# UCSB-NLP-Chang/Diffusion-SpaceTime-Attn

Measured on AMD Instinct MI355X. Metric: images/sec at 512x512, 50 PLMS steps, 2 objects, higher is better.
Workload: dtype fp16; 1 GPU; SD-v1-4 UNet+VAE (synthetic weights), 512x512, 50 PLMS steps (51 CFG UNet calls), 2 objects, fixed blend weights (BASELINE configs[1]); global_batch=64, parallelism=prompt-parallel dp1, hipgraph=True, linear_weights=fp16, trunk_layout=NHWC, weight_broadcast_bytes=0

## Files before the change

### diffusion-spacetime-attn_amd/csrc/sta_gemm.hip

```cpp

#include <hip/hip_runtime.h>
#include <stdint.h>
#include <type_traits>
#include "sta_xattn.h"
#include "sta_unet.h"
#include "sta_internal.h"
#include "sta_xattn_dev.h"

namespace {

constexpr int GM_NW = 8;
constexpr int GM_ROWS = 256;
constexpr int gm_part(int ntw) { return 32 * ntw; }
constexpr int gm_nt(int ntw) { return 2 * ntw; }
constexpr int gm_wfr(int ntw) { return 2 * gm_nt(ntw); }
constexpr int gm_wper(int ntw) { return (gm_wfr(ntw) + GM_NW - 1) / GM_NW; }
constexpr int gm_wslot(int ntw) { return gm_wper(ntw) * GM_NW * FRAG; }
constexpr int GM_XPER = 2 * (GM_ROWS / 16) / GM_NW;
constexpr int GM_XBUF = 2 * GM_ROWS * 64;
constexpr int gm_lds(int ntw) { return 2 * gm_wslot(ntw) + 2 * GM_XBUF; }

template <typename T>
__global__ __launch_bounds__(64) void pack_gemm_w_kernel(const T* __restrict__ w, long sn, long sk, T* __restrict__ packed, int nsteps, int nt) {
  const int fr = blockIdx.x;
  const int t = fr % nt, kci = (fr / nt) & 1, step = (fr / (2 * nt)) % nsteps, part = fr / (2 * nt * nsteps);
  const int lane = threadIdx.x, g = lane >> 4, c = lane & 15;
  const T* src = w + (size_t)(16 * nt * part + 16 * t + c) * sn + (size_t)(64 * step + 32 * kci + 8 * g) * sk;
  typename Tr<T>::V8 x;
#pragma unroll
  for (int j = 0; j < 8; ++j) x[j] = src[j * sk];
  *(typename Tr<T>::V8*)(packed + (size_t)fr * (FRAG / 2) + lane * 8) = x;
}

__device__ __forceinline__ float gm_row16_sum(float x) {
  x += __builtin_bit_cast(float, __builtin_amdgcn_update_dpp(0, __builtin_bit_cast(int, x), 0xB1, 0xf, 0xf, true));
  x += __builtin_bit_cast(float, __builtin_amdgcn_update_dpp(0, __builtin_bit_cast(int, x), 0x4E, 0xf, 0xf, true));
  x += __builtin_bit_cast(float, __builtin_amdgcn_update_dpp(0, __builtin_bit_cast(int, x), 0x141, 0xf, 0xf, true));
  x += __builtin_bit_cast(float, __builtin_amdgcn_update_dpp(0, __builtin_bit_cast(int, x), 0x140, 0xf, 0xf, true));
  return x;
}

struct GM {
  const char* x;
  const char* xb;
  int Ka;
  const char* w;
  const char* zeros;
  void* out;
  const void* bias;
  const void* res;
  float* stats;
  long rows_img;
  long R;
  int K, N, parts, items, xcd_map;
  long tiles;
};

template <typename T, int NTW>
__global__ __launch_bounds__(64 * GM_NW, 1) void gemm_rows_kernel(const GM p) {
  using V8 = typename Tr<T>::V8;
  using V4 = typename Tr<T>::V4;
  constexpr int PART = gm_part(NTW), NT = gm_nt(NTW), WFR = gm_wfr(NTW), WPER = gm_wper(NTW), WSLOT = gm_wslot(NTW);
  const int lane = threadIdx.x & 63;
  const int wv = __builtin_amdgcn_readfirstlane(threadIdx.x >> 6);
  const int g = lane >> 4, c16 = lane & 15;
  const int pq = wv & 3, ch = wv >> 2;
  char* xring = smem;
  char* wring = smem + 2 * GM_XBUF;
  const int nsteps = p.K >> 6;
  const __amdgpu_buffer_rsrc_t w_srd = make_srd(p.w, (unsigned)((size_t)p.parts * nsteps * WFR * FRAG));
  const unsigned lane16 = (unsigned)lane * 16u;

  auto item_tile = [&](int it, long& tile, int& part) {
    if (p.xcd_map) {
      const int j = it >> 3;
      tile = (long)(j / p.parts) * 8 + (it & 7);
      part = j % p.parts;
    } else {
      tile = it / p.parts;
      part = it - (int)tile * p.parts;
    }
  };
  const int nsteps_a = p.xb ? p.Ka >> 6 : nsteps;
  auto in_ptr = [&](long tile, int pc, bool second) -> const char* {
    const int rl = 16 * (pc & 15) + (lane >> 2);
    const long row = tile * GM_ROWS + rl;
    const int chunk = (lane & 3) ^ (((rl >> 2) & 1) << 1);
    const char* base = second ? p.xb + (size_t)row * (p.K - p.Ka) * sizeof(T) : p.x + (size_t)row * (p.xb ? p.Ka : p.K) * sizeof(T);
    return row < p.R ? base + (pc >> 4) * 64 + chunk * 16 : p.zeros + (pc >> 4) * 64 + chunk * 16;
  };
  auto stage_w = [&](int part, int step, int slot) __attribute__((always_inline)) {
    const unsigned base = (unsigned)((part * nsteps + step) * WFR) * (unsigned)FRAG;
#pragma unroll
    for (int i = 0; i < WPER; ++i) {
      const int f = wv + GM_NW * i;
      const int fs = f < WFR ? f : 0;
      __builtin_amdgcn_raw_ptr_buffer_load_lds(w_srd, (__attribute__((address_space(3))) void*)(wring + slot * WSLOT + f * FRAG), 16, lane16,
                                               base + (unsigned)fs * (unsigned)FRAG, 0, 0);
    }
  };
  auto stage_x = [&](const char* src, int pc, int buf) __attribute__((always_inline)) {
    __builtin_amdgcn_global_load_lds((const __attribute__((address_space(1))) void*)src,
                                     (__attribute__((address_space(3))) void*)(xring + buf * GM_XBUF + pc * FRAG), 16, 0, 0);
  };
  unsigned seg_e[4];
#pragma unroll
  for (int q = 0; q < 4; ++q) {
    const int rl = 64 * pq + 16 * q + c16;
    seg_e[q] = (unsigned)(rl * 64 + ((g ^ (((rl >> 2) & 1) << 1)) << 4));
  }

// ... 39 lines not shown
      auto stage_next = [&]() __attribute__((always_inline)) {
        if (!last) stage_w(part, st + 1, SL ^ 1);
        else if (more) stage_w(npart, 0, SL ^ 1);
        if (!last || more) {
#pragma unroll
          for (int i = 0; i < GM_XPER; ++i) {
            if (last) xp[i] = in_ptr(ntile, wv + GM_NW * i, false);
            else if (st + 1 == nsteps_a) xp[i] = in_ptr(tile, wv + GM_NW * i, true);
            stage_x(xp[i], wv + GM_NW * i, SL ^ 1);
            xp[i] += 128;
          }
        }
      };
      const char* xb = xring + SL * GM_XBUF;
      const V8* wf = (const V8*)(wring + SL * WSLOT + lane * 16) + (NTW * ch) * 64;
      V8 a[NTW], b[4];
      auto load_kc = [&](int kci, V8 (&aa)[NTW], V8 (&bb)[4]) __attribute__((always_inline)) {
#pragma unroll
        for (int q = 0; q < 4; ++q) bb[q] = *(const V8*)(xb + kci * (GM_ROWS * 64) + seg_e[q]);
#pragma unroll
        for (int t = 0; t < NTW; ++t) aa[t] = wf[(kci * NT + t) * 64];
      };
      load_kc(0, a, b);
#pragma unroll
      for (int kci = 0; kci < 2; ++kci) {
        V8 an[NTW], bn[4];
        if (kci < 1) load_kc(kci + 1, an, bn);
        __builtin_amdgcn_sched_barrier(0);
#pragma unroll
        for (int t = 0; t < NTW; ++t)
#pragma unroll
          for (int q = 0; q < 4; ++q) acc[q][t] = Tr<T>::mfma(a[t], b[q], acc[q][t]);
        __builtin_amdgcn_sched_barrier(0);
        if (kci == 0) {
          stage_next();
          __builtin_amdgcn_sched_barrier(0);
#pragma unroll
          for (int t = 0; t < NTW; ++t) a[t] = an[t];
#pragma unroll
          for (int q = 0; q < 4; ++q) b[q] = bn[q];
        }
      }
    };
    auto run_tile = [&](auto p0_tag) __attribute__((always_inline)) {
      constexpr int P0 = decltype(p0_tag)::value;
      for (int st = 0; st < nsteps; st += 2) {
        step(std::integral_constant<int, P0>{}, st);
        if (st + 1 < nsteps) step(std::integral_constant<int, P0 ^ 1>{}, st + 1);
      }
    };
    if (par == 0) run_tile(std::integral_constant<int, 0>{});
    else run_tile(std::integral_constant<int, 1>{});
    par ^= nsteps & 1;
    {
      typedef __attribute__((ext_vector_type(2))) unsigned u32x2;
      float bs[NTW][4];
#pragma unroll
      for (int t = 0; t < NTW; ++t) {
        V4 bv = {};
        if (p.bias) bv = *(const V4*)((const T*)p.bias + part * PART + ch * (16 * NTW) + 16 * t + 4 * g);
#pragma unroll
        for (int r = 0; r < 4; ++r) bs[t][r] = (float)bv[r];
      }
      float ssum[NTW][4], ssq[NTW][4];
#pragma unroll
      for (int t = 0; t < NTW; ++t)
#pragma unroll
        for (int r = 0; r < 4; ++r) { ssum[t][r] = 0.f; ssq[t][r] = 0.f; }
#pragma unroll
      for (int q = 0; q < 4; ++q) {
        const long row = tile * GM_ROWS + 64 * pq + 16 * q + c16;
        const bool ok = row < p.R;
        const unsigned base = (unsigned)(((size_t)row * p.N + part * PART + ch * (16 * NTW) + 4 * g) * sizeof(T));
        V4 rv[NTW];
        if (p.res) {
#pragma unroll
          for (int t = 0; t < NTW; ++t)
            rv[t] = __builtin_bit_cast(V4, __builtin_amdgcn_raw_buffer_load_b64(r_srd, ok ? base + (unsigned)(16 * t * sizeof(T)) : 0xfffffff0u, 0, 0));
        }
#pragma unroll
        for (int t = 0; t < NTW; ++t) {
          V4 o;
#pragma unroll
          for (int r = 0; r < 4; ++r) o[r] = (T)(acc[q][t][r] + bs[t][r] + (p.res ? (float)rv[t][r] : 0.f));
          __builtin_amdgcn_raw_buffer_store_b64(__builtin_bit_cast(u32x2, o), o_srd, ok ? base + (unsigned)(16 * t * sizeof(T)) : 0xfffffff0u, 0, 0);
          if (p.stats) {
#pragma unroll
            for (int r = 0; r < 4; ++r) {
              const float v = ok ? (float)o[r] : 0.f;
              ssum[t][r] += v;
              ssq[t][r] += v * v;
            }
          }
        }
      }
      if (p.stats) {
        const long row0 = tile * GM_ROWS;
        const bool live = row0 < p.R;
        const long img = live ? row0 / p.rows_img : p.R / p.rows_img;
        const int slot = live ? (int)((row0 - img * p.rows_img) / GM_ROWS) * 4 + pq : pq;
        const int slots = (int)(p.rows_img / GM_ROWS) * 4;
        float* dst = p.stats + (((size_t)img * slots + slot) * p.N + part * PART + ch * (16 * NTW) + 4 * g) * 2;
#pragma unroll
        for (int t = 0; t < NTW; ++t) {
          f32x4 lo, hi;
          lo[0] = gm_row16_sum(ssum[t][0]); lo[1] = gm_row16_sum(ssq[t][0]); lo[2] = gm_row16_sum(ssum[t][1]); lo[3] = gm_row16_sum(ssq[t][1]);
          hi[0] = gm_row16_sum(ssum[t][2]); hi[1] = gm_row16_sum(ssq[t][2]); hi[2] = gm_row16_sum(ssum[t][3]); hi[3] = gm_row16_sum(ssq[t][3]);
          if (c16 == 0) {
            *(f32x4*)(dst + 32 * t) = lo;
            *(f32x4*)(dst + 32 * t + 4) = hi;
          }
        }
      }
    }
    if (!more) break;
    it = nit; tile = ntile; part = npart;
    first_of_tile = true;
  }
  asm volatile("s_waitcnt vmcnt(0)" ::: "memory");
}

}

extern "C" {

static int gemm_ntw(int N) { return N > 0 && N % 160 == 0 ? 5 : (N > 0 && N % 128 == 0 ? 4 : 0); }

int sta_linear_rows_supported(long R, int K, int N) {
  if (R <= 0 || K <= 0 || K % 64 || gemm_ntw(N) == 0) return 0;
  if ((size_t)R * N * 2 >= 0xfffffff0ull) return 0;
  return 1;
}

size_t sta_linear_rows_packed_w_bytes(int K, int N) { return (K > 0 && K % 64 == 0 && gemm_ntw(N)) ? (size_t)N * K * 2 : 0; }

int sta_linear_rows_pack_w(const void* w, long sn, long sk, void* packed, int K, int N, int dtype, void* stream) {
  g_sta_err[0] = 0;
  if (!w || !packed) return sta_fail(STA_E_ARG, "null pointer");
  if (sta_linear_rows_packed_w_bytes(K, N) == 0) return sta_fail(STA_E_UNSUP, "linear_rows: K %% 64 == 0 and N %% 160 == 0 or N %% 128 == 0 (K=%d N=%d)", K, N);
  hipStream_t st = (hipStream_t)stream;
  const int nsteps = K / 64, nt = gm_nt(gemm_ntw(N));
  const unsigned nfr = (unsigned)(N / (16 * nt)) * nsteps * 2 * nt;
  return sta_by_dtype(dtype, [&](auto tag) {
    using T = decltype(tag);
    return sta_launch<pack_gemm_w_kernel<T>>("pack_gemm_w launch", dim3(nfr), dim3(64), 0, st, (const T*)w, sn, sk, (T*)packed, nsteps, nt);
  });
}

static int linear_rows_impl(const void* x, const void* xb, int Ka, const void* packed_w, const void* zeros, const void* bias, const void* res,
                            void* out, long R, int K, int N, int dtype, void* stream, float* stats = nullptr, long rows_img = 0) {
  g_sta_err[0] = 0;
  if (!x || !packed_w || !zeros || !out) return sta_fail(STA_E_ARG, "null pointer");
  if (xb && (Ka <= 0 || Ka >= K || Ka % 64)) return sta_fail(STA_E_ARG, "linear_rows_cat: Ka=%d of K=%d (need 0 < Ka < K, Ka %% 64 == 0)", Ka, K);
  if (!sta_linear_rows_supported(R, K, N)) return sta_fail(STA_E_UNSUP, "linear_rows: unsupported shape R=%ld K=%d N=%d", R, K, N);
  if (dtype != STA_BF16 && dtype != STA_F16) return sta_fail(STA_E_UNSUP, "dtype %d", dtype);
  const int ntw = gemm_ntw(N);
  if (stats && (rows_img <= 0 || rows_img % GM_ROWS || R % rows_img)) return sta_fail(STA_E_ARG, "linear_rows_stats: rows_per_image=%ld (need a multiple of 256 dividing R=%ld)", rows_img, R);
  GM p{(const char*)x, (const char*)xb, Ka, (const char*)packed_w, (const char*)zeros, out, bias, res, stats, rows_img, R, K, N, N / gm_part(ntw), 0, 0, (R + GM_ROWS - 1) / GM_ROWS};
  const long items = p.tiles * p.parts;
  if (items >= (1l << 30)) return sta_fail(STA_E_UNSUP, "linear_rows: too many tiles");
  p.items = (int)items;
  p.xcd_map = p.tiles % 8 == 0;
  const unsigned grid = (unsigned)(p.items < 256 ? p.items : 256);
  hipStream_t st = (hipStream_t)stream;
  return sta_by_dtype(dtype, [&](auto tag) {
    using T = decltype(tag);
    const char* const what = "linear_rows launch";
    if (ntw == 5) return sta_launch_lds<gemm_rows_kernel<T, 5>>(what, gm_lds(5), dim3(grid), dim3(64 * GM_NW), gm_lds(5), st, p);
    return sta_launch_lds<gemm_rows_kernel<T, 4>>(what, gm_lds(4), dim3(grid), dim3(64 * GM_NW), gm_lds(4), st, p);
  });
}

int sta_linear_rows(const void* x, const void* packed_w, const void* zeros, const void* bias, const void* res, void* out, long R, int K, int N,
                    int dtype, void* stream) {
  return linear_rows_impl(x, nullptr, 0, packed_w, zeros, bias, res, out, R, K, N, dtype, stream);
}

int sta_linear_rows_stats(const void* x, const void* packed_w, const void* zeros, const void* bias, const void* res, void* out, float* stats,
                          long rows_per_image, long R, int K, int N, int dtype, void* stream) {
  if (!stats) { g_sta_err[0] = 0; return sta_fail(STA_E_ARG, "null pointer"); }
  return linear_rows_impl(x, nullptr, 0, packed_w, zeros, bias, res, out, R, K, N, dtype, stream, stats, rows_per_image);
}

int sta_linear_rows_cat(const void* xa, const void* xb, int Ka, const void* packed_w, const void* zeros, const void* bias, const void* res,
                        void* out, long R, int K, int N, int dtype, void* stream) {
  if (!xb) { g_sta_err[0] = 0; return sta_fail(STA_E_ARG, "null pointer"); }
  return linear_rows_impl(xa, xb, Ka, packed_w, zeros, bias, res, out, R, K, N, dtype, stream);
}

}
```

### diffusion-spacetime-attn_amd/sta/fused.py

```python

import torch

from . import lib

_DT = {torch.bfloat16: lib.STA_BF16, torch.float16: lib.STA_F16}
ENABLED = True
_hold = 0
TRACKED = False


class held:

    def __enter__(self):
        global _hold
        _hold += 1

    def __exit__(self, *exc):
        global _hold
        _hold -= 1


class tracked:

    def __init__(self, on=True):
# ... 365 lines not shown
    if n_post.shape != (B, 4, Hh, Ww) or n_enc.shape != (B, 4, Hh, Ww):
        raise ValueError("vae_encode_step: noises must be [B, 4, h, w] = %s" % ((B, 4, Hh, Ww),))
    x = torch.empty((B, 4, Hh, Ww), dtype=torch.float32, device=h.device)
    z0 = torch.empty_like(x) if want_z0 else None
    xin = torch.empty((2 * B, 4, Hh, Ww), dtype=h.dtype, device=h.device) if want_xin else None
    lib.check(lib.load().sta_vae_encode_step(h.data_ptr(), qw.data_ptr(), qb.data_ptr(), n_post.data_ptr(), n_enc.data_ptr(), x.data_ptr(),
                                             _ptr(z0), _ptr(xin), B, Hh * Ww, float(scale_factor), float(sqrt_a), float(sqrt_1ma), _DT[h.dtype],
                                             _stream()), "sta_vae_encode_step")
    return x, z0, xin


CAT_IN_PLACE = True


def groupnorm_silu_cat(xa, xb, weight, bias, groups, eps, silu=True):
    B, Ca = xa.shape[0], xa.shape[1]
    C = Ca + xb.shape[1]
    HW = xa.numel() // (B * Ca)
    L = lib.load()
    y = torch.empty((B, C) + tuple(xa.shape[2:]), dtype=xa.dtype, device=xa.device, memory_format=torch.channels_last)
    sa, sb = (_producer_stats(xa), _producer_stats(xb)) if GN_STATS_FROM_PRODUCER else (None, None)
    if sa is not None and sb is not None:
        lib.check(L.sta_groupnorm_silu_nhwc_cstats(xa.data_ptr(), xb.data_ptr(), Ca, sa.data_ptr(), sb.data_ptr(), None, weight.data_ptr(),
                                                   bias.data_ptr(), y.data_ptr(), B, C, HW, groups, float(eps), int(bool(silu)), _DT[xa.dtype],
                                                   _stream()), "sta_groupnorm_silu_nhwc_cstats")
        return y
    ws = torch.empty(L.sta_groupnorm_nhwc_workspace_bytes(B, HW, groups) // 4, dtype=torch.float32, device=xa.device)
    lib.check(L.sta_groupnorm_silu_nhwc_cat(xa.data_ptr(), xb.data_ptr(), Ca, None, weight.data_ptr(), bias.data_ptr(), y.data_ptr(),
                                            ws.data_ptr(), B, C, HW, groups, float(eps), int(bool(silu)), _DT[xa.dtype], _stream()),
              "sta_groupnorm_silu_nhwc_cat")
    return y


def cat_supported(xa, xb, groups, skip_weight):
    if not (CAT_IN_PLACE and usable(xa) and is_nhwc(xa) and is_nhwc(xb) and xa.dtype == xb.dtype and xa.shape[0] == xb.shape[0]
            and xa.shape[2:] == xb.shape[2:]):
        return False
    Ca, C = xa.shape[1], xa.shape[1] + xb.shape[1]
    if Ca % 64 or C % 8 or C % groups or (C // groups < 8 and C // groups != 4) or C > 4096 or groups > 64:
        return False
    rows = xa.numel() // Ca
    return (LINEAR_ROWS and rows >= LINEAR_MIN_ROWS and skip_weight.dtype == xa.dtype
            and bool(lib.load().sta_linear_rows_supported(rows, C, skip_weight.shape[0])))


def linear_rows_cat(xa, xb, w_packed, N, bias=None, res=None):
    Ka, Kb = xa.shape[-1], xb.shape[-1]
    R = xa.numel() // Ka
    assert xa.is_contiguous() and xb.is_contiguous() and xb.numel() // Kb == R and Ka % 64 == 0
    out = torch.empty(xa.shape[:-1] + (N,), dtype=xa.dtype, device=xa.device)
    if bias is not None:
        bias = bias.to(xa.dtype).contiguous()
    z = _zeros_page(xa.device, 2 * (Ka + Kb))
    lib.check(lib.load().sta_linear_rows_cat(xa.data_ptr(), xb.data_ptr(), Ka, w_packed.data_ptr(), z.data_ptr(), _ptr(bias), _ptr(res),
                                             out.data_ptr(), R, Ka + Kb, N, _DT[xa.dtype], _stream()), "sta_linear_rows_cat")
    return out


LINEAR_ROWS = True
LINEAR_MIN_ROWS = 4096


_retired_pages = []


def _zeros_page(device, nbytes):
    z = _conv_zeros.get(device)
    if z is None or z.numel() < nbytes:
        if z is not None:
            _retired_pages.append(z)
        z = _conv_zeros[device] = torch.zeros(max(nbytes, 16384), dtype=torch.uint8, device=device)
    return z


def linear_rows_supported(x, weight):
    if not (LINEAR_ROWS and x.is_cuda and x.dtype in _DT and not torch.is_grad_enabled() and ENABLED and not _hold and weight.dtype == x.dtype):
        return False
    K = x.shape[-1]
    R = x.numel() // K
    return R >= LINEAR_MIN_ROWS and x.is_contiguous() and bool(lib.load().sta_linear_rows_supported(R, K, weight.shape[0]))


def pack_linear_weight(weight):
    N, K = weight.shape[0], weight.shape[1]
    L = lib.load()
    n = L.sta_linear_rows_packed_w_bytes(K, N)
    if n == 0 or not weight.is_cuda:
        raise ValueError("linear_rows: a CUDA weight [N %% 160 == 0 or N %% 128 == 0, K %% 64 == 0]; got %s" % (tuple(weight.shape),))
    w = weight.detach()
    buf = torch.empty(n, dtype=torch.uint8, device=w.device)
    lib.check(L.sta_linear_rows_pack_w(w.data_ptr(), w.stride(0), w.stride(1), buf.data_ptr(), K, N, _DT[w.dtype], _stream()), "sta_linear_rows_pack_w")
    return buf


def linear_rows(x, w_packed, N, bias=None, res=None, stats_rows=None):
    K = x.shape[-1]
    R = x.numel() // K
    out = torch.empty(x.shape[:-1] + (N,), dtype=x.dtype, device=x.device)
    if res is not None:
        assert res.numel() == out.numel() and res.dtype == x.dtype and res.is_contiguous()
    if bias is not None:
        bias = bias.to(x.dtype).contiguous()
    z = _zeros_page(x.device, 2 * K)
    if stats_rows and stats_rows % 256 == 0 and R % stats_rows == 0:
        n_img, slots = R // stats_rows, stats_rows // 64
        part = torch.empty((n_img + 1, slots, N, 2), dtype=torch.float32, device=x.device)
        lib.check(lib.load().sta_linear_rows_stats(x.data_ptr(), w_packed.data_ptr(), z.data_ptr(), _ptr(bias), _ptr(res), out.data_ptr(),
                                                   part.data_ptr(), stats_rows, R, K, N, _DT[x.dtype], _stream()), "sta_linear_rows_stats")
        if _version(out) is not None:
            out._sta_stats = (out._version, _finalize_stats(part, n_img, slots, N))
        return out
    lib.check(lib.load().sta_linear_rows(x.data_ptr(), w_packed.data_ptr(), z.data_ptr(), _ptr(bias), _ptr(res), out.data_ptr(), R, K, N,
                                         _DT[x.dtype], _stream()), "sta_linear_rows")
    return out


def packed_linear_weight(owner, key_obj, weight):
    key = (weight.data_ptr(), _version(weight), weight.dtype)
    cache = owner.__dict__.setdefault("_sta_linear_cache", {})
    hit = cache.get(id(key_obj))
    if hit is None or hit[0] != key:
        hit = cache[id(key_obj)] = (key, pack_linear_weight(weight))
    return hit[1]


def linear_module(lin, x, res=None):
    if linear_rows_supported(x, lin.weight) and (res is None or res.is_contiguous()):
        return linear_rows(x, packed_linear_weight(lin, lin, lin.weight), lin.weight.shape[0], bias=lin.bias, res=res)
    y = torch.nn.functional.linear(x, lin.weight, lin.bias)
    return y if res is None else y + res


def add_bias_nchw(a, b=None, bias=None):
    B, C = a.shape[0], a.shape[1]
    HW = a.numel() // (B * C)
    if (C % 8 if is_nhwc(a) else HW % 8):
        t = a if b is None else a + b
        return t if bias is None else t + bias[None, :, None, None]
    y = torch.empty_like(a)
    if is_nhwc(a):
        if b is not None and not is_nhwc(b):
            b = b.contiguous(memory_format=torch.channels_last)
        lib.check(lib.load().sta_add_bias_rows(a.data_ptr(), _ptr(b), _ptr(bias), y.data_ptr(), B * HW, C, _DT[a.dtype], _stream()),
                  "sta_add_bias_rows")
        return y
    if b is not None and not b.is_contiguous():
        b = b.contiguous()
    lib.check(lib.load().sta_add_bias_nchw(a.data_ptr(), _ptr(b), _ptr(bias), y.data_ptr(), B, C, HW, _DT[a.dtype], _stream()),
              "sta_add_bias_nchw")
    return y


def tracked_usable(x):
    return (TRACKED and ENABLED and x.is_cuda and x.dtype in _DT and torch.is_grad_enabled()
            and (is_nhwc(x) if x.dim() == 4 else x.is_contiguous()))

# ... 150 lines not shown
```

### diffusion-spacetime-attn_amd/sta/lib.py

```python
import ctypes
import os
import shutil
import subprocess

_HERE = os.path.dirname(os.path.abspath(__file__))
PKG_ROOT = os.path.dirname(_HERE)
REPO_ROOT = os.path.dirname(PKG_ROOT)
CSRC = os.path.join(PKG_ROOT, "csrc")
INCLUDE = os.path.join(REPO_ROOT, "include")
LIB_PATH = os.path.join(CSRC, "libsta_xattn.so")
SOURCES = [os.path.join(CSRC, n) for n in ("sta_xattn.hip", "sta_xattn_bwd.hip", "sta_xattn_proj.hip", "sta_xattn_proj3.hip", "sta_rowgemm.hip", "sta_ffgemm.hip", "sta_lnqkv.hip", "sta_conv.hip", "sta_gemm.hip", "sta_selfattn.hip", "sta_selfattn_bwd.hip", "sta_unet.hip", "sta_unet_bwd.hip", "sta_fp8.hip", "sta_mxfp8.hip", "sta_sampler.hip", "sta_encode.hip", "sta_clip.hip", "sta_inpaint.hip")]

PER_SOURCE_FLAGS = {"sta_selfattn.hip": ["-mllvm", "-amdgpu-mfma-vgpr-form", "-ffinite-math-only"],
                    "sta_selfattn_bwd.hip": ["-mllvm", "-amdgpu-mfma-vgpr-form", "-ffinite-math-only"],
                    "sta_xattn.hip": ["-ffinite-math-only"], "sta_xattn_bwd.hip": ["-ffinite-math-only"], "sta_xattn_proj.hip": ["-ffinite-math-only"],
                    "sta_xattn_proj3.hip": ["-ffinite-math-only"], "sta_rowgemm.hip": ["-ffinite-math-only"], "sta_ffgemm.hip": ["-ffinite-math-only"], "sta_conv.hip": ["-ffinite-math-only"], "sta_gemm.hip": ["-ffinite-math-only"]}

STA_BF16, STA_F16 = 0, 1
STA_MX8_GEGLU, STA_MX8_MX_OUT = 1, 2
OPT_FWD_KERNEL, OPT_STAGED_TILES, OPT_STAGED_WAVES, OPT_STAGED_QT, OPT_HEAD_MAJOR, OPT_SPLIT_QT, OPT_SELFATTN_32, OPT_PROJ_PAIR, OPT_SELFATTN_WAVES, OPT_SELFATTN_PIPE, OPT_PROJ_LL2, OPT_BWD_KERNEL, OPT_BWD_SLOTS, OPT_BWD_WAVES = range(14)
FWD_STAGED, FWD_SPLIT = 1, 2
MAX_KEYS, MAX_HEAD_DIM, MAX_OBJECTS = 80, 160, 8
P3_STATS_WORDS = 8

_vp, _i, _f, _sz, _l = ctypes.c_void_p, ctypes.c_int, ctypes.c_float, ctypes.c_size_t, ctypes.c_long
SYMBOLS = {
    "sta_version": (_i, []),
    "sta_last_error": (ctypes.c_char_p, []),
    "sta_built_with": (ctypes.c_char_p, []),
    "sta_set_option": (_i, [_i, _i]),
    "sta_xattn_packed_kv_bytes": (_sz, [_i, _i, _i]),
    "sta_xattn_pack_kv": (_i, [_vp, _vp, _vp, _i, _i, _i, _i, _i, _vp]),
    "sta_xattn_fwd": (_i, [_vp, _vp, _vp, _vp, _vp, _vp, _i, _i, _i, _i, _i, _i, _f, _i, _vp]),
    "sta_xattn_fwd_proj_supported": (_i, [_i, _i, _i, _i]),
    "sta_xattn_fwd_proj_locals_from_l2": (_i, [_i, _i, _i, _i]),
    "sta_xattn_packed_wq_bytes": (_sz, [_i, _i]),
    "sta_xattn_pack_wq": (_i, [_vp, _vp, _i, _i, _i, _vp]),
    "sta_xattn_packed_kv_proj_bytes": (_sz, [_i, _i, _i]),
    "sta_xattn_pack_kv_proj": (_i, [_vp, _vp, _vp, _i, _i, _i, _i, _i, _vp]),
    "sta_xattn_fwd_proj": (_i, [_vp, _vp, _vp, _vp, _vp, _vp, _i, _i, _i, _i, _i, _i, _f, _i, _vp]),
    "sta_xattn_fwd_proj_qfrag_supported": (_i, [_i, _i, _i, _i, _i, _i]),
    "sta_xattn_fwd_proj_ex": (_i, [_vp, _vp, _vp, _vp, _vp, _vp, _i, _i, _i, _i, _i, _i, _f, _i, _i, _vp, _vp]),
    "sta_xattn_fwd_proj_qfrag": (_i, [_vp, _vp, _vp, _vp, _vp, _vp, _i, _i, _i, _i, _i, _i, _f, _i, _vp]),
    "sta_xattn_fwd_proj_qfrag_ofrag": (_i, [_vp, _vp, _vp, _vp, _vp, _vp, _i, _i, _i, _i, _i, _i, _f, _i, _vp]),
    "sta_to_out_ln_packed_wo_bytes": (_sz, [_i, _i]),
    "sta_to_out_ln_pack_wo": (_i, [_vp, _vp, _i, _i, _i, _i, _vp]),
    "sta_to_out_ln_ofrag": (_i, [_vp, _vp, _vp, _vp, _vp, _vp, _vp, _vp, _l, _i, _i, _f, _i, _i, _vp]),
    "sta_selfattn_fwd_sfrag": (_i, [_vp, _vp, _vp, _vp, _i, _i, _i, _i, _i, _i, _l, _l, _f, _i, _vp]),
    "sta_xattn_bwd_workspace_bytes": (_sz, [_i, _i, _i, _i]),
    "sta_xattn_bwd": (_i, [_vp, _vp, _vp, _vp, _vp, _vp, _vp, _vp, _i, _i, _i, _i, _i, _i, _f, _i, _vp]),
    "sta_selfattn_fwd": (_i, [_vp, _vp, _vp, _vp, _i, _i, _i, _i, _i, _i, _l, _l, _f, _i, _vp]),
    "sta_selfattn_fwd_optimistic": (_i, [_vp, _vp, _vp, _vp, _vp, _i, _i, _i, _i, _i, _i, _l, _l, _f, _i, _i, _vp]),
    "sta_selfattn_optimistic_supported": (_i, [_i, _i, _i, _f, _i]),
    "sta_selfattn_optimistic_flags_bytes": (ctypes.c_size_t, [_i, _i, _i]),
    "sta_selfattn_fwd_lse": (_i, [_vp, _vp, _vp, _vp, _vp, _i, _i, _i, _i, _i, _i, _l, _l, _f, _i, _vp]),
    "sta_selfattn_bwd": (_i, [_vp] * 13 + [_i, _i, _i, _i, _i, _i, _f, _i, _vp]),
    "sta_groupnorm_silu": (_i, [_vp, _vp, _vp, _vp, _vp, _i, _i, _i, _i, _f, _i, _i, _vp]),
    "sta_geglu": (_i, [_vp, _vp, _l, _i, _i, _vp]),
    "sta_add_layernorm": (_i, [_vp, _vp, _vp, _vp, _vp, _vp, _vp, _l, _i, _f, _i, _vp]),
    "sta_add_layernorm_qfrag": (_i, [_vp, _vp, _vp, _vp, _vp, _vp, _vp, _l, _i, _f, _i, _vp]),
    "sta_ff_geglu_packed_w_bytes": (_sz, [_i, _i]),
    "sta_ff_geglu_pack_w": (_i, [_vp, _vp, _i, _i, _i, _vp]),
    "sta_ff_geglu_qfrag": (_i, [_vp, _vp, _vp, _vp, _l, _i, _i, _i, _i, _vp]),
    "sta_ff_out_packed_w_bytes": (_sz, [_i, _i]),
    "sta_ff_out_pack_w": (_i, [_vp, _vp, _i, _i, _i, _vp]),
    "sta_ff_out_res_hfrag": (_i, [_vp, _vp, _vp, _vp, _vp, _l, _i, _i, _i, _vp]),
    "sta_ln_qkv_packed_w_bytes": (_sz, [_i]),
    "sta_ln_qkv_pack_w": (_i, [_vp, _vp, _vp, _i, _i, _vp]),
    "sta_ln_qkv": (_i, [_vp] * 9 + [_l, _i, _f, _i, _vp]),
    "sta_conv3x3_nhwc_supported": (_i, [_i, _i, _i, _i, _i]),
    "sta_conv3x3_packed_w_bytes": (_sz, [_i, _i]),
    "sta_conv3x3_pack_w": (_i, [_vp, _l, _l, _l, _l, _vp, _i, _i, _i, _vp]),
    "sta_conv3x3_nhwc": (_i, [_vp, _vp, _vp, _vp, _vp, _vp, _vp, _i, _i, _i, _i, _i, _i, _i, _vp]),
# ... 188 lines not shown
```

### include/sta_xattn.h

```cpp
#ifndef STA_XATTN_H
#define STA_XATTN_H

#include <stddef.h>
#include <stdint.h>

#ifdef __cplusplus
extern "C" {
#endif

#define STA_VERSION 0x000500

enum { STA_BF16 = 0, STA_F16 = 1 };

enum {
  STA_OK = 0,
  STA_E_ARG = -1,
  STA_E_UNSUP = -2,
  STA_E_LAUNCH = -3
};

#define STA_MAX_KEYS 80
#define STA_MAX_HEAD_DIM 160
#define STA_MAX_OBJECTS 8

const char* sta_built_with(void);

int sta_version(void);

const char* sta_last_error(void);

enum {
  STA_OPT_FWD_KERNEL = 0,
  STA_OPT_STAGED_TILES = 1,
  STA_OPT_STAGED_WAVES = 2,
  STA_OPT_STAGED_QT = 3,
  STA_OPT_HEAD_MAJOR = 4,
  STA_OPT_SPLIT_QT = 5,
  STA_OPT_SELFATTN_32 = 6,
  STA_OPT_PROJ_PAIR = 7,
  STA_OPT_SELFATTN_WAVES = 8,
  STA_OPT_SELFATTN_PIPE = 9,
  STA_OPT_PROJ_LL2 = 10,
  STA_OPT_BWD_KERNEL = 11,
  STA_OPT_BWD_SLOTS = 12,
  STA_OPT_BWD_WAVES = 13,
  STA_OPT_COUNT = 14
};
int sta_set_option(int key, int value);

size_t sta_xattn_packed_kv_bytes(int n_ctx, int heads, int d);

int sta_xattn_pack_kv(const void* k, const void* v, void* packed,
                      int n_ctx, int M, int C, int heads, int dtype, void* stream);

int sta_xattn_fwd(const void* q, const void* packed, const uint8_t* mask, const float* coef,
                  void* out, float* maps,
                  int n_img, int N, int C, int heads, int M, int K, float scale, int dtype, void* stream);

int sta_xattn_fwd_proj_supported(int C, int heads, int M, int K);
size_t sta_xattn_packed_wq_bytes(int C, int heads);
int sta_xattn_pack_wq(const void* wq, void* packed, int C, int heads, int dtype, void* stream);
size_t sta_xattn_packed_kv_proj_bytes(int n_ctx, int heads, int d);
int sta_xattn_pack_kv_proj(const void* k, const void* v, void* packed,
                           int n_ctx, int M, int C, int heads, int dtype, void* stream);
int sta_xattn_fwd_proj(const void* y, const void* packed_wq, const void* packed_kv, const uint8_t* mask,
                       const float* coef, void* out,
                       int n_img, int N, int C, int heads, int M, int K, float scale, int dtype, void* stream);
int sta_xattn_fwd_proj_locals_from_l2(int C, int heads, int M, int K);

int sta_xattn_fwd_proj_qfrag_supported(int n_img, int N, int C, int heads, int M, int K);
int sta_xattn_fwd_proj_qfrag(const void* y_frag, const void* packed_wq, const void* packed_kv, const uint8_t* mask,
                             const float* coef, void* out,
                             int n_img, int N, int C, int heads, int M, int K, float scale, int dtype, void* stream);

int sta_xattn_fwd_proj_qfrag_ofrag(const void* y_frag, const void* packed_wq, const void* packed_kv, const uint8_t* mask,
                                   const float* coef, void* out_frag,
                                   int n_img, int N, int C, int heads, int M, int K, float scale, int dtype, void* stream);

#define STA_P3_STATS_WORDS 8
int sta_xattn_fwd_proj_ex(const void* y, const void* packed_wq, const void* packed_kv, const uint8_t* mask,
                          const float* coef, void* out,
                          int n_img, int N, int C, int heads, int M, int K, float scale, int dtype, int layout, void* stats, void* stream);
size_t sta_to_out_ln_packed_wo_bytes(int C, int heads);
int sta_to_out_ln_pack_wo(const void* wo, void* packed, int C, int heads, int kind, int dtype, void* stream);
int sta_to_out_ln_ofrag(const void* blended_ofrag, const void* packed_wo, const void* bias, const void* x,
                        const void* gamma, const void* beta, void* s, void* y,
                        long R, int C, int heads, float eps, int y_qfrag, int dtype, void* stream);
int sta_selfattn_fwd_sfrag(const void* q, const void* k, const void* vt, void* out_frag, int B, int N, int C, int heads,
                           int ldq, int ldk, long vt_row_stride, long vt_batch_stride, float scale, int dtype, void* stream);

size_t sta_xattn_bwd_workspace_bytes(int n_img, int N, int heads, int K);

int sta_xattn_bwd(const void* q, const void* packed, const uint8_t* mask, const float* coef,
                  const void* dout, void* dq, float* dcoef, void* workspace,
                  int n_img, int N, int C, int heads, int M, int K, float scale, int dtype, void* stream);

int sta_selfattn_fwd(const void* q, const void* k, const void* vt, void* out, int B, int N, int C, int heads,
                     int ldq, int ldk, long vt_row_stride, long vt_batch_stride, float scale, int dtype, void* stream);

// ... 17 lines not shown
```

Baseline: 9.397 images/s.

## Add triple-buffered ring row-GEMM kernel prefetching across tiles and epilogue

Adds a new row GEMM kernel with a three-slot input ring and a two-slot weight ring. It keeps loads in flight across tile boundaries, so the next item's operands are staged while the current tile finishes and its epilogue runs. Bias and residual loads are issued early, during the last K step, instead of in the epilogue. Python enables this kernel by default through a new option, and an optional mode remaps tiles to the full grid. The cost is more LDS per block and more complex vmcnt bookkeeping.

Measured after the change: 9.457 images/s, median of 6. Within noise of the previous version (+0.6%).

```diff
diff --git a/diffusion-spacetime-attn_amd/csrc/sta_gemm.hip b/diffusion-spacetime-attn_amd/csrc/sta_gemm.hip
--- a/diffusion-spacetime-attn_amd/csrc/sta_gemm.hip
+++ b/diffusion-spacetime-attn_amd/csrc/sta_gemm.hip
@@ -19,6 +19,7 @@
 constexpr int GM_XPER = 2 * (GM_ROWS / 16) / GM_NW;
 constexpr int GM_XBUF = 2 * GM_ROWS * 64;
 constexpr int gm_lds(int ntw) { return 2 * gm_wslot(ntw) + 2 * GM_XBUF; }
+constexpr int gm_lds_ring(int ntw) { return 2 * gm_wslot(ntw) + 3 * GM_XBUF; }
 
 template <typename T>
 __global__ __launch_bounds__(64) void pack_gemm_w_kernel(const T* __restrict__ w, long sn, long sk, T* __restrict__ packed, int nsteps, int nt) {
@@ -57,6 +58,80 @@
 };
 
 template <typename T, int NTW>
+__device__ __forceinline__ unsigned gm_out_offset(const GM& p, long tile, int part, int pq, int ch, int g, int c16, int q) {
+  const long row = tile * GM_ROWS + 64 * pq + 16 * q + c16;
+  return row < p.R ? (unsigned)(((size_t)row * p.N + part * gm_part(NTW) + ch * (16 * NTW) + 4 * g) * sizeof(T)) : 0xfffffff0u;
+}
+
+template <typename T, int NTW, bool PRE>
+__device__ __forceinline__ void gm_epilogue(const GM& p, const f32x4 (&acc)[4][NTW], const typename Tr<T>::V4 (*rv_pre)[NTW], const typename Tr<T>::V4* bv_pre, long tile, int part, int pq,
+                                            int ch, int g, int c16, __amdgpu_buffer_rsrc_t o_srd, __amdgpu_buffer_rsrc_t r_srd) {
+  using V4 = typename Tr<T>::V4;
+  constexpr int PART = gm_part(NTW);
+  typedef __attribute__((ext_vector_type(2))) unsigned u32x2;
+  float bs[NTW][4];
+#pragma unroll
+  for (int t = 0; t < NTW; ++t) {
+    V4 bv = {};
+    if constexpr (PRE) bv = bv_pre[t];
+    else if (p.bias) bv = *(const V4*)((const T*)p.bias + part * PART + ch * (16 * NTW) + 16 * t + 4 * g);
+#pragma unroll
+    for (int r = 0; r < 4; ++r) bs[t][r] = (float)bv[r];
+  }
+  float ssum[NTW][4], ssq[NTW][4];
+#pragma unroll
+  for (int t = 0; t < NTW; ++t)
+#pragma unroll
+    for (int r = 0; r < 4; ++r) { ssum[t][r] = 0.f; ssq[t][r] = 0.f; }
+#pragma unroll
+  for (int q = 0; q < 4; ++q) {
+    const unsigned base = gm_out_offset<T, NTW>(p, tile, part, pq, ch, g, c16, q);
+    const bool ok = base != 0xfffffff0u;
+    V4 rv[NTW];
+    if (p.res) {
+#pragma unroll
+      for (int t = 0; t < NTW; ++t) {
+        if constexpr (PRE) rv[t] = rv_pre[q][t];
+        else rv[t] = __builtin_bit_cast(V4, __builtin_amdgcn_raw_buffer_load_b64(r_srd, ok ? base + (unsigned)(16 * t * sizeof(T)) : 0xfffffff0u, 0, 0));
+      }
+    }
+#pragma unroll
+    for (int t = 0; t < NTW; ++t) {
+      V4 o;
+#pragma unroll
+      for (int r = 0; r < 4; ++r) o[r] = (T)(acc[q][t][r] + bs[t][r] + (p.res ? (float)rv[t][r] : 0.f));
+      __builtin_amdgcn_raw_buffer_store_b64(__builtin_bit_cast(u32x2, o), o_srd, ok ? base + (unsigned)(16 * t * sizeof(T)) : 0xfffffff0u, 0, 0);
+      if (p.stats) {
+#pragma unroll
+        for (int r = 0; r < 4; ++r) {
+          const float v = ok ? (float)o[r] : 0.f;
+          ssum[t][r] += v;
+          ssq[t][r] += v * v;
+        }
+      }
+    }
+  }
+  if (p.stats) {
+    const long row0 = tile * GM_ROWS;
+    const bool live = row0 < p.R;
+    const long img = live ? row0 / p.rows_img : p.R / p.rows_img;
+    const int slot = live ? (int)((row0 - img * p.rows_img) / GM_ROWS) * 4 + pq : pq;
+    const int slots = (int)(p.rows_img / GM_ROWS) * 4;
+    float* dst = p.stats + (((size_t)img * slots + slot) * p.N + part * PART + ch * (16 * NTW) + 4 * g) * 2;
+#pragma unroll
+    for (int t = 0; t < NTW; ++t) {
+      f32x4 lo, hi;
+      lo[0] = gm_row16_sum(ssum[t][0]); lo[1] = gm_row16_sum(ssq[t][0]); lo[2] = gm_row16_sum(ssum[t][1]); lo[3] = gm_row16_sum(ssq[t][1]);
+      hi[0] = gm_row16_sum(ssum[t][2]); hi[1] = gm_row16_sum(ssq[t][2]); hi[2] = gm_row16_sum(ssum[t][3]); hi[3] = gm_row16_sum(ssq[t][3]);
+      if (c16 == 0) {
+        *(f32x4*)(dst + 32 * t) = lo;
+        *(f32x4*)(dst + 32 * t + 4) = hi;
+      }
+    }
+  }
+}
+
+template <typename T, int NTW>
 __global__ __launch_bounds__(64 * GM_NW, 1) void gemm_rows_kernel(const GM p) {
   using V8 = typename Tr<T>::V8;
   using V4 = typename Tr<T>::V4;
@@ -202,72 +277,202 @@
     if (par == 0) run_tile(std::integral_constant<int, 0>{});
     else run_tile(std::integral_constant<int, 1>{});
     par ^= nsteps & 1;
-    {
-      typedef __attribute__((ext_vector_type(2))) unsigned u32x2;
-      float bs[NTW][4];
-#pragma unroll
-      for (int t = 0; t < NTW; ++t) {
-        V4 bv = {};
-        if (p.bias) bv = *(const V4*)((const T*)p.bias + part * PART + ch * (16 * NTW) + 16 * t + 4 * g);
-#pragma unroll
-        for (int r = 0; r < 4; ++r) bs[t][r] = (float)bv[r];
-      }
-      float ssum[NTW][4], ssq[NTW][4];
-#pragma unroll
-      for (int t = 0; t < NTW; ++t)
-#pragma unroll
-        for (int r = 0; r < 4; ++r) { ssum[t][r] = 0.f; ssq[t][r] = 0.f; }
-#pragma unroll
-      for (int q = 0; q < 4; ++q) {
-        const long row = tile * GM_ROWS + 64 * pq + 16 * q + c16;
-        const bool ok = row < p.R;
-        const unsigned base = (unsigned)(((size_t)row * p.N + part * PART + ch * (16 * NTW) + 4 * g) * sizeof(T));
-        V4 rv[NTW];
-        if (p.res) {
-#pragma unroll
-          for (int t = 0; t < NTW; ++t)
-            rv[t] = __builtin_bit_cast(V4, __builtin_amdgcn_raw_buffer_load_b64(r_srd, ok ? base + (unsigned)(16 * t * sizeof(T)) : 0xfffffff0u, 0, 0));
-        }
-#pragma unroll
-        for (int t = 0; t < NTW; ++t) {
-          V4 o;
-#pragma unroll
-          for (int r = 0; r < 4; ++r) o[r] = (T)(acc[q][t][r] + bs[t][r] + (p.res ? (float)rv[t][r] : 0.f));
-          __builtin_amdgcn_raw_buffer_store_b64(__builtin_bit_cast(u32x2, o), o_srd, ok ? base + (unsigned)(16 * t * sizeof(T)) : 0xfffffff0u, 0, 0);
-          if (p.stats) {
-#pragma unroll
-            for (int r = 0; r < 4; ++r) {
-              const float v = ok ? (float)o[r] : 0.f;
-              ssum[t][r] += v;
-              ssq[t][r] += v * v;
-            }
-          }
-        }
-      }
-      if (p.stats) {
-        const long row0 = tile * GM_ROWS;
-        const bool live = row0 < p.R;
-        const long img = live ? row0 / p.rows_img : p.R / p.rows_img;
-        const int slot = live ? (int)((row0 - img * p.rows_img) / GM_ROWS) * 4 + pq : pq;
-        const int slots = (int)(p.rows_img / GM_ROWS) * 4;
-        float* dst = p.stats + (((size_t)img * slots + slot) * p.N + part * PART + ch * (16 * NTW) + 4 * g) * 2;
-#pragma unroll
-        for (int t = 0; t < NTW; ++t) {
-          f32x4 lo, hi;
-          lo[0] = gm_row16_sum(ssum[t][0]); lo[1] = gm_row16_sum(ssq[t][0]); lo[2] = gm_row16_sum(ssum[t][1]); lo[3] = gm_row16_sum(ssq[t][1]);
-          hi[0] = gm_row16_sum(ssum[t][2]); hi[1] = gm_row16_sum(ssq[t][2]); hi[2] = gm_row16_sum(ssum[t][3]); hi[3] = gm_row16_sum(ssq[t][3]);
-          if (c16 == 0) {
-            *(f32x4*)(dst + 32 * t) = lo;
-            *(f32x4*)(dst + 32 * t + 4) = hi;
-          }
-        }
-      }
-    }
+    gm_epilogue<T, NTW, false>(p, acc, nullptr, nullptr, tile, part, pq, ch, g, c16, o_srd, r_srd);
     if (!more) break;
     it = nit; tile = ntile; part = npart;
     first_of_tile = true;
   }
   asm volatile("s_waitcnt vmcnt(0)" ::: "memory");
+}
+
+template <int N>
+__device__ __forceinline__ void gm_wait_vm() { asm volatile("s_waitcnt vmcnt(%0)" ::"n"(N) : "memory"); }
+
+struct GmCur {
+  int it;
+  long tile;
+  int part, st;
+  bool valid;
+};
+
+template <typename T, int NTW>
+__global__ __launch_bounds__(64 * GM_NW, 1) void gemm_rows_ring_kernel(const GM p) {
+  using V8 = typename Tr<T>::V8;
+  using V4 = typename Tr<T>::V4;
+  constexpr int NT = gm_nt(NTW), WFR = gm_wfr(NTW), WPER = gm_wper(NTW), WSLOT = gm_wslot(NTW);
+  constexpr int EPI = 4 * NTW, EPI_STATS = 4 * NTW + 2 * NTW;
+  const int lane = threadIdx.x & 63;
+  const int wv = __builtin_amdgcn_readfirstlane(threadIdx.x >> 6);
+  const int g = lane >> 4, c16 = lane & 15;
+  const int pq = wv & 3, ch = wv >> 2;
+  char* xring = smem;
+  char* wring = smem + 3 * GM_XBUF;
+  const int nsteps = p.K >> 6;
+  const int nsteps_a = p.xb ? p.Ka >> 6 : nsteps;
+  const __amdgpu_buffer_rsrc_t w_srd = make_srd(p.w, (unsigned)((size_t)p.parts * nsteps * WFR * FRAG));
+  const unsigned lane16 = (unsigned)lane * 16u;
+
+  auto item_tile = [&](int it, long& tile, int& part) {
+    if (p.xcd_map == 2) {
+      const int j = it / (int)gridDim.x;
+      tile = (long)(j / p.parts) * gridDim.x + it % (int)gridDim.x;
+      part = j % p.parts;
+    } else if (p.xcd_map) {
+      const int j = it >> 3;
+      tile = (long)(j / p.parts) * 8 + (it & 7);
+      part = j % p.parts;
+    } else {
+      tile = it / p.parts;
+      part = it - (int)tile * p.parts;
+    }
+  };
+  auto advance = [&](GmCur c) -> GmCur {
+    if (!c.valid) return c;
+    if (++c.st < nsteps) return c;
+    c.st = 0;
+    c.it += gridDim.x;
+    c.valid = c.it < p.items;
+    if (c.valid) item_tile(c.it, c.tile, c.part);
+    return c;
+  };
+  auto in_ptr = [&](long tile, int pc, bool second) -> const char* {
+    const int rl = 16 * (pc & 15) + (lane >> 2);
+    const long row = tile * GM_ROWS + rl;
+    const int chunk = (lane & 3) ^ (((rl >> 2) & 1) << 1);
+    const char* base = second ? p.xb + (size_t)row * (p.K - p.Ka) * sizeof(T) : p.x + (size_t)row * (p.xb ? p.Ka : p.K) * sizeof(T);
+    return row < p.R ? base + (pc >> 4) * 64 + chunk * 16 : p.zeros + (pc >> 4) * 64 + chunk * 16;
+  };
+  const char* xp[GM_XPER];
+  auto retarget = [&](const GmCur& from, const GmCur& to) __attribute__((always_inline)) {
+    if (!to.valid) return;
+#pragma unroll
+    for (int i = 0; i < GM_XPER; ++i) {
+      if (to.st == 0) xp[i] = in_ptr(to.tile, wv + GM_NW * i, false);
+      else if (to.st == nsteps_a) xp[i] = in_ptr(to.tile, wv + GM_NW * i, true);
+      else xp[i] += 128;
+    }
+    (void)from;
+  };
+  auto stage_w = [&](const GmCur& c, int slot) __attribute__((always_inline)) {
+    const unsigned base = (unsigned)((c.part * nsteps + c.st) * WFR) * (unsigned)FRAG;
+#pragma unroll
+    for (int i = 0; i < WPER; ++i) {
+      const int f = wv + GM_NW * i;
+      const int fs = f < WFR ? f : 0;
+      __builtin_amdgcn_raw_ptr_buffer_load_lds(w_srd, (__attribute__((address_space(3))) void*)(wring + slot * WSLOT + f * FRAG), 16, lane16,
+                                               base + (unsigned)fs * (unsigned)FRAG, 0, 0);
+    }
+  };
+  auto stage_x = [&](int slot) __attribute__((always_inline)) {
+#pragma unroll
+    for (int i = 0; i < GM_XPER; ++i)
+      __builtin_amdgcn_global_load_lds((const __attribute__((address_space(1))) void*)xp[i],
+                                       (__attribute__((address_space(3))) void*)(xring + slot * GM_XBUF + (wv + GM_NW * i) * FRAG), 16, 0, 0);
+  };
+  unsigned seg_e[4];
+#pragma unroll
+  for (int q = 0; q < 4; ++q) {
+    const int rl = 64 * pq + 16 * q + c16;
+    seg_e[q] = (unsigned)(rl * 64 + ((g ^ (((rl >> 2) & 1) << 1)) << 4));
+  }
+
+  GmCur c0{(int)blockIdx.x, 0, 0, 0, (int)blockIdx.x < p.items};
+  if (!c0.valid) return;
+  item_tile(c0.it, c0.tile, c0.part);
+#pragma unroll
+  for (int i = 0; i < GM_XPER; ++i) xp[i] = in_ptr(c0.tile, wv + GM_NW * i, false);
+  stage_w(c0, 0);
+  stage_x(0);
+  GmCur c1 = advance(c0);
+  retarget(c0, c1);
+  if (c1.valid) stage_x(1);
+  GmCur c2 = advance(c1);
+  retarget(c1, c2);
+  int xs = 0, ws = 0;
+
+  const size_t obytes = (size_t)p.R * p.N * sizeof(T);
+  const __amdgpu_buffer_rsrc_t o_srd = make_srd(p.out, (unsigned)(obytes < 0xfffffff0ull ? obytes : 0xfffffff0ull));
+  const __amdgpu_buffer_rsrc_t r_srd = make_srd(p.res ? p.res : p.out, (unsigned)(obytes < 0xfffffff0ull ? obytes : 0xfffffff0ull));
+  bool first_of_item = false;
+
+  while (true) {
+    f32x4 acc[4][NTW];
+#pragma unroll
+    for (int q = 0; q < 4; ++q)
+#pragma unroll
+      for (int t = 0; t < NTW; ++t) acc[q][t] = f32x4{0.f, 0.f, 0.f, 0.f};
+    V4 rv[4][NTW] = {}, bv[NTW] = {};
+    const long tile = c0.tile;
+    const int part = c0.part;
+
+    for (int st = 0; st < nsteps; ++st) {
+      if (first_of_item) {
+        if (p.stats) { if (c1.valid) gm_wait_vm<GM_XPER + EPI_STATS>(); else gm_wait_vm<EPI_STATS>(); }
+        else { if (c1.valid) gm_wait_vm<GM_XPER + EPI>(); else gm_wait_vm<EPI>(); }
+      } else {
+        if (c1.valid) gm_wait_vm<GM_XPER>(); else gm_wait_vm<0>();
+      }
+      first_of_item = false;
+      __builtin_amdgcn_s_barrier();
+      const int xs2 = xs == 0 ? 2 : xs - 1;
+      GmCur c3 = c2;
+      auto stage_next = [&]() __attribute__((always_inline)) {
+        if (c1.valid) stage_w(c1, ws ^ 1);
+        if (c2.valid) stage_x(xs2);
+        c3 = advance(c2);
+        retarget(c2, c3);
+        if (st + 1 == nsteps && p.bias) {
+#pragma unroll
+          for (int t = 0; t < NTW; ++t) bv[t] = *(const V4*)((const T*)p.bias + part * gm_part(NTW) + ch * (16 * NTW) + 16 * t + 4 * g);
+        }
+        if (st + 1 == nsteps && p.res) {
+#pragma unroll
+          for (int q = 0; q < 4; ++q) {
+            const unsigned base = gm_out_offset<T, NTW>(p, tile, part, pq, ch, g, c16, q);
+#pragma unroll
+            for (int t = 0; t < NTW; ++t)
+              rv[q][t] = __builtin_bit_cast(V4, __builtin_amdgcn_raw_buffer_load_b64(r_srd, base != 0xfffffff0u ? base + (unsigned)(16 * t * sizeof(T)) : base, 0, 0));
+          }
+        }
+      };
+      const char* xb = xring + xs * GM_XBUF;
+      const V8* wf = (const V8*)(wring + ws * WSLOT + lane * 16) + (NTW * ch) * 64;
+      V8 a[NTW], b[4];
+      auto load_kc = [&](int kci, V8 (&aa)[NTW], V8 (&bb)[4]) __attribute__((always_inline)) {
+#pragma unroll
+        for (int q = 0; q < 4; ++q) bb[q] = *(const V8*)(xb + kci * (GM_ROWS * 64) + seg_e[q]);
+#pragma unroll
+        for (int t = 0; t < NTW; ++t) aa[t] = wf[(kci * NT + t) * 64];
+      };
+      load_kc(0, a, b);
+#pragma unroll
+      for (int kci = 0; kci < 2; ++kci) {
+        V8 an[NTW], bn[4];
+        if (kci < 1) load_kc(kci + 1, an, bn);
+        __builtin_amdgcn_sched_barrier(0);
+#pragma unroll
+        for (int t = 0; t < NTW; ++t)
+#pragma unroll
+          for (int q = 0; q < 4; ++q) acc[q][t] = Tr<T>::mfma(a[t], b[q], acc[q][t]);
+        __builtin_amdgcn_sched_barrier(0);
+        if (kci == 0) {
+          stage_next();
+          __builtin_amdgcn_sched_barrier(0);
+#pragma unroll
+          for (int t = 0; t < NTW; ++t) a[t] = an[t];
+#pragma unroll
+          for (int q = 0; q < 4; ++q) b[q] = bn[q];
+        }
+      }
+      c0 = c1; c1 = c2; c2 = c3;
+      xs = xs == 2 ? 0 : xs + 1;
+      ws ^= 1;
+    }
+    gm_epilogue<T, NTW, true>(p, acc, rv, bv, tile, part, pq, ch, g, c16, o_srd, r_srd);
+    if (!c0.valid) break;
+    first_of_item = true;
+  }
+  gm_wait_vm<0>();
 }
 
 }
@@ -313,6 +518,15 @@
   p.xcd_map = p.tiles % 8 == 0;
   const unsigned grid = (unsigned)(p.items < 256 ? p.items : 256);
   hipStream_t st = (hipStream_t)stream;
+  const int mode = g_sta_opt[STA_OPT_ROWGEMM_RING];
+  if (mode == 3 && p.parts > 1 && grid == 256 && p.tiles % 256 == 0) p.xcd_map = 2;
+  if (mode != 2)
+    return sta_by_dtype(dtype, [&](auto tag) {
+      using T = decltype(tag);
+      const char* const what = "linear_rows launch";
+      if (ntw == 5) return sta_launch_lds<gemm_rows_ring_kernel<T, 5>>(what, gm_lds_ring(5), dim3(grid), dim3(64 * GM_NW), gm_lds_ring(5), st, p);
+      return sta_launch_lds<gemm_rows_ring_kernel<T, 4>>(what, gm_lds_ring(4), dim3(grid), dim3(64 * GM_NW), gm_lds_ring(4), st, p);
+    });
   return sta_by_dtype(dtype, [&](auto tag) {
     using T = decltype(tag);
     const char* const what = "linear_rows launch";
diff --git a/diffusion-spacetime-attn_amd/sta/fused.py b/diffusion-spacetime-attn_amd/sta/fused.py
--- a/diffusion-spacetime-attn_amd/sta/fused.py
+++ b/diffusion-spacetime-attn_amd/sta/fused.py
@@ -441,6 +441,7 @@
     if bias is not None:
         bias = bias.to(xa.dtype).contiguous()
     z = _zeros_page(xa.device, 2 * (Ka + Kb))
+    _rowgemm_switch()
     lib.check(lib.load().sta_linear_rows_cat(xa.data_ptr(), xb.data_ptr(), Ka, w_packed.data_ptr(), z.data_ptr(), _ptr(bias), _ptr(res),
                                              out.data_ptr(), R, Ka + Kb, N, _DT[xa.dtype], _stream()), "sta_linear_rows_cat")
     return out
@@ -448,6 +449,12 @@
 
 LINEAR_ROWS = True
 LINEAR_MIN_ROWS = 4096
+ROWGEMM_RING = True
+
+
+def _rowgemm_switch():
+    if (lib.get_option(lib.OPT_ROWGEMM_RING) == 2) == ROWGEMM_RING:
+        lib.set_option(lib.OPT_ROWGEMM_RING, 0 if ROWGEMM_RING else 2)
 
 
 _retired_pages = []
@@ -491,6 +498,7 @@
     if bias is not None:
         bias = bias.to(x.dtype).contiguous()
     z = _zeros_page(x.device, 2 * K)
+    _rowgemm_switch()
     if stats_rows and stats_rows % 256 == 0 and R % stats_rows == 0:
         n_img, slots = R // stats_rows, stats_rows // 64
         part = torch.empty((n_img + 1, slots, N, 2), dtype=torch.float32, device=x.device)
diff --git a/diffusion-spacetime-attn_amd/sta/lib.py b/diffusion-spacetime-attn_amd/sta/lib.py
--- a/diffusion-spacetime-attn_amd/sta/lib.py
+++ b/diffusion-spacetime-attn_amd/sta/lib.py
@@ -18,7 +18,7 @@
 
 STA_BF16, STA_F16 = 0, 1
 STA_MX8_GEGLU, STA_MX8_MX_OUT = 1, 2
-OPT_FWD_KERNEL, OPT_STAGED_TILES, OPT_STAGED_WAVES, OPT_STAGED_QT, OPT_HEAD_MAJOR, OPT_SPLIT_QT, OPT_SELFATTN_32, OPT_PROJ_PAIR, OPT_SELFATTN_WAVES, OPT_SELFATTN_PIPE, OPT_PROJ_LL2, OPT_BWD_KERNEL, OPT_BWD_SLOTS, OPT_BWD_WAVES = range(14)
+OPT_FWD_KERNEL, OPT_STAGED_TILES, OPT_STAGED_WAVES, OPT_STAGED_QT, OPT_HEAD_MAJOR, OPT_SPLIT_QT, OPT_SELFATTN_32, OPT_PROJ_PAIR, OPT_SELFATTN_WAVES, OPT_SELFATTN_PIPE, OPT_PROJ_LL2, OPT_BWD_KERNEL, OPT_BWD_SLOTS, OPT_BWD_WAVES, OPT_ROWGEMM_RING = range(15)
 FWD_STAGED, FWD_SPLIT = 1, 2
 MAX_KEYS, MAX_HEAD_DIM, MAX_OBJECTS = 80, 160, 8
 P3_STATS_WORDS = 8
diff --git a/include/sta_xattn.h b/include/sta_xattn.h
--- a/include/sta_xattn.h
+++ b/include/sta_xattn.h
@@ -44,7 +44,8 @@
   STA_OPT_BWD_KERNEL = 11,
   STA_OPT_BWD_SLOTS = 12,
   STA_OPT_BWD_WAVES = 13,
-  STA_OPT_COUNT = 14
+  STA_OPT_ROWGEMM_RING = 14,
+  STA_OPT_COUNT = 15
 };
 int sta_set_option(int key, int value);
 
```
